# OmerMersin/video-stab

Hardware: AMD Instinct MI355X
Metric: stabilized frames/sec @1080p (whole job; warp-stage HBM GB/s in roofline) (higher is better)
Workload: dtype u8

## Files before the change

### video-stab_amd/csrc/batch_schedule.cpp

```cpp
#include <cstring>
#include <new>

#include "stab_internal.h"

using namespace vsd;

struct vs_batch {
    int device = 0, S = 0, B = 0, cap = 0;
    bool own = false;
    std::vector<vs_stab*> m;
    vs_stab* ref = nullptr;
    std::string err;
    FirstFailure failure;
    hipStream_t st = nullptr, st_pre = nullptr, st_det = nullptr, st_up = nullptr;
    bool allocated = false;
    uint8_t* h_tables = nullptr;
    size_t h_set_bytes = 0, ho_pairs = 0, ho_lk = 0, ho_rs = 0, ho_tail = 0, ho_gf = 0, ho_seg = 0;
    uint8_t* d_all = nullptr;
    uint8_t *d_lk[2] = {nullptr, nullptr}, *d_rs[2] = {nullptr, nullptr}, *d_tail[2] = {nullptr, nullptr}, *d_seg[2] = {nullptr, nullptr}, *d_gf = nullptr;
    uint8_t* d_tin[2] = {nullptr, nullptr};
    ImgPair* d_pairs[2] = {nullptr, nullptr};
    size_t up_bytes = 0;
    int pre_rel_step = -1;
    double* d_MinvB[2] = {nullptr, nullptr};
    int32_t* d_tabs[2] = {nullptr, nullptr};
    int tab_ints = 0;
    hipEvent_t ev_bpre = nullptr, ev_bgray = nullptr, ev_bnms = nullptr, ev_bdet[4] = {}, ev_blk[4] = {}, ev_warp[2] = {}, ev_rel[2] = {}, ev_up[2] = {}, ev_go = nullptr;
    bool bdet_valid[4] = {false, false, false, false}, warp_valid[2] = {false, false}, rel_valid[2] = {false, false};
    int last_det_batch = -1, last_warp_set = -1, batch_id = 0, pend_set = 0;
    struct Ready {
        bool valid = false, tabs_built = false;
        int n = 0, set = 0, step = -1;
        size_t stride = 0;
        std::vector<const uint8_t*> srcs;
        std::vector<uint8_t*> dsts;
        std::vector<int> slots, pad_idx;
        std::vector<vs_stab*> owner;
    };
    static constexpr int NRQ = WARP_LAG + 1;
    Ready rq[NRQ];
    int rq_head = 0, rq_n = 0;
    Ready& pending(int i) { return rq[(rq_head + i) % NRQ]; }
    Ready& building() { return rq[(rq_head + rq_n) % NRQ]; }
    void pop_pending() { rq_head = (rq_head + 1) % NRQ; rq_n--; }

    struct HostSet { uint8_t* base; ImgPair* pairs; uint8_t *lk, *rs, *tail, *seg, *gf; };
    HostSet host_set(int k) const {
        uint8_t* b = h_tables + (size_t)(k % 4) * h_set_bytes;
        return {b, reinterpret_cast<ImgPair*>(b + ho_pairs), b + ho_lk, b + ho_rs, b + ho_tail, b + ho_seg, b + ho_gf};
    }
    int dev_set(int k) const { return k & 1; }
    hipEvent_t blk_event(int k) const { return ev_blk[k % 4]; }
    hipEvent_t det_event(int k) const { return ev_bdet[k % 4]; }
    bool& det_valid(int k) { return bdet_valid[k % 4]; }
    static_assert(WARP_LAG >= 1 && WARP_LAG <= 2, "d_MinvB / d_tabs / ev_warp / ev_rel: two sets cover a lag of at most two steps");
    void flip_pend_set() { pend_set ^= 1; }
    bool warps_due(int k) { return rq_n > 0 && pending(0).step <= k - WARP_LAG; }

    template <typename F>
    void each_event(F f) {
        for (hipEvent_t* e : {&ev_bpre, &ev_bgray, &ev_bnms, &ev_warp[0], &ev_warp[1], &ev_rel[0], &ev_rel[1], &ev_up[0], &ev_up[1], &ev_go}) f(*e);
        for (auto& e : ev_bdet) f(e);
        for (auto& e : ev_blk) f(e);
    }
};

namespace {

void group_free(vs_batch* g) {
    if (g->h_tables) (void)hipHostFree(g->h_tables);
    if (g->d_all) (void)hipFree(g->d_all);
    g->h_tables = nullptr; g->d_all = nullptr;
    g->allocated = false;
    g->ref = nullptr;
}

bool group_make_events(vs_batch* g) {
    bool ok = true;
    g->each_event([&](hipEvent_t& e) { ok = ok && hipEventCreateWithFlags(&e, hipEventDisableTiming) == hipSuccess; });
    return ok;
}

static bool same_yuv_pad(const vs_stab* a, const vs_stab* b) {
    const bool on = yuv_pad_on(a);
    if (on != yuv_pad_on(b)) return false;
    if (!on) return true;
    const vs_yuv_fill x = yuv_pad_fill(a), y = yuv_pad_fill(b);
    return x.y == y.y && x.u == y.u && x.v == y.v;
}
static bool same_yuv_edge_fill(const vs_stab* a, const vs_stab* b) {
    const bool on = yuv_edge_fill_on(a);
    if (on != yuv_edge_fill_on(b)) return false;
    if (!on) return true;
    const vs_yuv_fill x = yuv_edge_fill(a), y = yuv_edge_fill(b);
    return x.y == y.y && x.u == y.u && x.v == y.v;
}
bool same_launch_shape(const vs_stab* a, const vs_stab* b) {
    const vs_params_c &p = a->p, &q = b->p;
    return a->w == b->w && a->h == b->h && a->fmt == b->fmt && a->src_pitch == b->src_pitch && a->zero_copy == b->zero_copy &&
           a->in == b->in && a->out == b->out && a->yuv_cz == b->yuv_cz && same_yuv_pad(a, b) && same_yuv_edge_fill(a, b) &&
           a->aw == b->aw && a->ah == b->ah && a->levels == b->levels &&
           p.lk_win_size == q.lk_win_size && p.ransac_max_iters == q.ransac_max_iters && p.border_size == q.border_size &&
           p.crop_n_zoom == q.crop_n_zoom && (p.border_size <= 0 || p.border_type == q.border_type);
}

int group_allocate(vs_batch* g) {
    const vs_stab* s0 = g->ref;
    const int cap = g->cap, ngf = g->S * (g->B / 2 + 1);
    size_t off = 0;
    auto take = [&](size_t bytes) { size_t o = off; off += (bytes + 255) & ~(size_t)255; return o; };
    const size_t o_gf = take(gftt_item_bytes() * ngf);
    size_t ho = 0;
    auto htake = [&](size_t bytes) { size_t o = ho; ho += (bytes + 255) & ~(size_t)255; return o; };
    g->ho_pairs = htake(sizeof(ImgPair) * cap * MAX_PYR);
    g->ho_lk = htake(lk_item_bytes() * cap); g->ho_rs = htake(ransac_item_bytes() * cap);
    g->ho_tail = htake(tail_item_bytes() * cap); g->ho_seg = htake(tail_seg_bytes() * g->S);
    g->up_bytes = ho;
    g->ho_gf = htake(gftt_item_bytes() * ngf);
    g->h_set_bytes = ho;
    const size_t o_set[2] = {take(g->up_bytes), take(g->up_bytes)};
    const size_t o_ti[2] = {take(tail_in_bytes() * cap), take(tail_in_bytes() * cap)};
    const size_t o_minv[2] = {take((size_t)cap * 96), take((size_t)cap * 96)};
    int tow, toh;
    out_size(s0, s0->w, s0->h, &tow, &toh);
    g->tab_ints = s0->pf->three_planes() ? planar_tab_ints(tow, toh, s0->pf->sx, s0->pf->sy) : s0->pf->luma_uv() ? nv12_tab_ints(tow, toh) : (int)warp_tabs_ints(std::max(s0->w, tow), std::max(s0->h, toh), 1);
    size_t o_tabs[2];
    for (auto& o : o_tabs) o = take((size_t)g->tab_ints * cap * sizeof(int32_t));
    VS_OBJ_HIP(g, hipMalloc((void**)&g->d_all, off));
    VS_OBJ_HIP(g, hipMemsetAsync(g->d_all, 0, off, g->st));
    uint8_t* b = g->d_all;
    g->d_gf = b + o_gf;
    for (int i = 0; i < 2; i++) {
        uint8_t* ds = b + o_set[i];
        g->d_pairs[i] = (ImgPair*)(ds + g->ho_pairs);
        g->d_lk[i] = ds + g->ho_lk; g->d_rs[i] = ds + g->ho_rs; g->d_tail[i] = ds + g->ho_tail; g->d_seg[i] = ds + g->ho_seg; g->d_tin[i] = b + o_ti[i];
        g->d_MinvB[i] = (double*)(b + o_minv[i]);
    }
    for (int i = 0; i < 2; i++) g->d_tabs[i] = (int32_t*)(b + o_tabs[i]);
    VS_OBJ_HIP(g, hipHostMalloc((void**)&g->h_tables, 4 * ho));
    memset(g->h_tables, 0, 4 * ho);
    VS_OBJ_HIP(g, hipStreamSynchronize(g->st));
    for (vs_batch::Ready& r : g->rq) {
        r.srcs.assign(cap, nullptr); r.dsts.assign(cap, nullptr); r.slots.assign(cap, -1); r.pad_idx.assign(cap, 0); r.owner.assign(cap, nullptr);
    }
    g->allocated = true;
    return VS_OK;
}

struct WarpEnds { const uint8_t* src; uint8_t* dst; };
WarpEnds warp_ends(const vs_stab* o, const uint8_t* frame, uint8_t* d_out, int pad_idx, const BorderPlan& bp) {
    if (!bp.pad && !bp.crop) return {frame, d_out};
    return bp.pad ? WarpEnds{scratch(o, pad_idx), d_out} : WarpEnds{frame, scratch(o, pad_idx)};
}

int group_ready_launches(vs_batch* g, vs_batch::Ready& R, int what, hipStream_t st) {
    const vs_stab* s0 = g->ref;
    const BorderPlan bp = border_plan(s0);
    const bool cz = yuv_cz_on(s0);
    const bool yp = yuv_pad_on(s0);
    const YuvBorder wb = s0->pf->kind != PIX_INTERLEAVED ? yuv_warp_border(s0) : YuvBorder{VS_BORDER_BLACK, WarpFill()};
    int rc = VS_OK;
    for (int i0 = 0; i0 < R.n && rc == VS_OK; i0 += WARP_BATCH_MAX) {
        const int m = std::min(WARP_BATCH_MAX, R.n - i0);
        const uint8_t* srcs[WARP_BATCH_MAX];
        uint8_t* dsts[WARP_BATCH_MAX];
        for (int i = 0; i < m; i++) {
            const WarpEnds e = warp_ends(R.owner[i0 + i], R.srcs[i0 + i], R.dsts[i0 + i], R.pad_idx[i0 + i], bp);
            srcs[i] = e.src; dsts[i] = e.dst;
            if (bp.pad && !yp && what != VS_WARP_TABLES_ONLY && rc == VS_OK)
                rc = launch_make_border(R.srcs[i0 + i], s0->src_pitch, s0->w, s0->h, s0->cn, const_cast<uint8_t*>(e.src), bp.prow, bp.b, s0->p.border_type, st);
        }
        if (yp && what != VS_WARP_TABLES_ONLY && rc == VS_OK) rc = pad_launch(s0, &R.srcs[i0], const_cast<uint8_t* const*>(srcs), m, st);
        if (rc != VS_OK) break;
        const WarpMaps maps{g->d_MinvB[R.set] + 12 * i0, 12, false};
        const WarpTabs tabs{WarpTabs::CALLER, g->d_tabs[R.set] + (size_t)i0 * g->tab_ints, g->tab_ints, what};
        if (s0->pf->kind != PIX_INTERLEAVED) {
            rc = warp_yuv(srcs, dsts, m, warp_src_planes(s0), warp_dst_planes(s0, dsts[0], R.stride), maps, wb, tabs, st);
            if (cz && what != VS_WARP_TABLES_ONLY && rc == VS_OK) rc = cz_launch(s0, dsts, &R.dsts[i0], m, R.stride, st);
            continue;
        }
        rc = launch_warp_plane(srcs, dsts, m, bp.pad ? bp.prow : s0->src_pitch, bp.pw, bp.ph, bp.crop ? bp.prow : R.stride, bp.pw, bp.ph, s0->cn, maps,
                               VS_BORDER_BLACK, tabs, st);
        for (int i = 0; bp.crop && what != VS_WARP_TABLES_ONLY && i < m && rc == VS_OK; i++)
            rc = launch_resize_linear(dsts[i] + ((size_t)bp.b * s0->w + bp.b) * s0->cn, bp.prow, s0->w - 2 * bp.b, s0->h - 2 * bp.b, s0->cn,
                                      R.dsts[i0 + i], R.stride, R.owner[i0 + i]->orig_w, R.owner[i0 + i]->orig_h, st);
    }
    if (rc != VS_OK) g->err = get_last_error();
    return rc;
}

int group_launch_ready(vs_batch* g, hipEvent_t det_done = nullptr) {
    if (g->rq_n == 0) return VS_OK;
    vs_batch::Ready& R = g->pending(0);
    hipStream_t st = g->st_pre;
    int rc;
    if (g->rel_valid[R.set] || det_done) {
        hipError_t e = hipSuccess;
        if (WARP_LAG >= 2) {
            if (g->rel_valid[R.set]) e = hipStreamWaitEvent(st, g->ev_rel[R.set], 0);
            if (e == hipSuccess && det_done) e = hipStreamWaitEvent(st, det_done, 0);
        } else {
            if (det_done) e = hipStreamWaitEvent(g->st_up, det_done, 0);
            if (e == hipSuccess && g->rel_valid[R.set]) e = hipStreamWaitEvent(g->st_up, g->ev_rel[R.set], 0);
            if (e == hipSuccess) e = hipEventRecord(g->ev_go, g->st_up);
            if (e == hipSuccess) e = hipStreamWaitEvent(st, g->ev_go, 0);
        }
        if (e != hipSuccess) return vs_obj_fail(g, VS_ERR_HIP, "hipStreamWaitEvent failed");
        if (g->rel_valid[R.set]) g->pre_rel_step = std::max(g->pre_rel_step, R.step);
        g->rel_valid[R.set] = false;
    }
    {
        StageScope t(g->ref, VS_STAGE_WARP, st);
        rc = group_ready_launches(g, R, R.tabs_built ? VS_WARP_ONLY : VS_WARP_ALL, st);
    }
    const hipError_t ew = hipEventRecord(g->ev_warp[R.set], st);
    if (ew == hipSuccess) { g->warp_valid[R.set] = true; g->last_warp_set = R.set; }
    else if (rc == VS_OK) rc = hip_fail(ew, "hipEventRecord(g->ev_warp[R.set], st)");
    for (int i = 0; i < R.n; i++) {
        if (!R.owner[i]) continue;
        const int rrc = release_slot(R.owner[i], R.slots[i], st);
        if (rc == VS_OK) rc = rrc;
    }
    R.valid = false;
    g->pop_pending();
    if (rc != VS_OK) g->err = get_last_error();
    return rc;
}


struct StepPlan {
    int k = 0;
    int n = 0, max_n = 0;
    int n_max = 0;
    int ndet = 0;
    int npend = 0, nseg = 0;
    int aligned = 1;
    int any_apart = 0, all_apart = 1;
    size_t pend_stride = 0;
};

int fill_stream_items(vs_batch* g, vs_stab* s, const vs_batch::HostSet& H, const BorderPlan& bp, int ndue, int first, StepPlan& P) {
    const vs_params_c& p = s->p;
    const int ns = (int)s->bq.size(), dset = g->dev_set(P.k), set = g->pend_set;
    vs_batch::Ready& R = g->building();
    int npad = 0;
    for (int i = 0; i < ns; i++) {
        const int idx = first + i;
        const vs_stab::BFrame& b = s->bq[i];
        const vs_stab::ItemBufs& it = s->items[i];
        LKLevel L[MAX_PYR];
        fill_lk_levels(s, b.pv, b.c, L);
        const int cap = std::max(b.lk_cap, 0);
        P.n_max = std::max(P.n_max, cap);
        uint8_t *rs = H.rs + ransac_item_bytes() * idx, *tail = H.tail + tail_item_bytes() * idx;
        VS_OBJ_TRY(g, lk_fill_item(H.lk + lk_item_bytes() * idx, L, s->levels, s->d_pts[b.lk_buf], cap, s->d_npts[b.lk_buf], it.next, it.status, it.err,
                              p.lk_win_size, p.lk_max_iters, p.lk_epsilon));
        VS_OBJ_TRY(g, ransac_fill_item(rs, s->d_pts[b.lk_buf], it.next, it.status, cap, s->d_npts[b.lk_buf], it.vp, it.vc, it.m, 4, p.ransac_threshold,
                                  p.ransac_max_iters, s->tab, it.counts, it.model, it.inliers, it.info, s->d_traj, &s->tp, s->d_dbg, b.have_prev_gray));
        ransac_item_set_last(rs, i == ns - 1 ? 1 : 0);
        ransac_item_set_tail_in(rs, g->d_tin[dset] + tail_in_bytes() * idx);
        double* minv = nullptr;
        WarpTabJob jobs[2] = {{nullptr, nullptr, nullptr, 0, 0}, {nullptr, nullptr, nullptr, 0, 0}};
        if (b.out_due) {
            const int j = P.npend++;
            minv = g->d_MinvB[set] + 12 * j;
            R.srcs[j] = b.out_frame; R.dsts[j] = b.d_out; R.slots[j] = b.out_slot; R.owner[j] = s; R.pad_idx[j] = npad;
            if (P.all_apart && std::min(WARP_BATCH_MAX, ndue - j / WARP_BATCH_MAX * WARP_BATCH_MAX) >= WARP_TAB_MIN) {
                const WarpEnds e = warp_ends(s, b.out_frame, b.d_out, npad, bp);
                int32_t* T = g->d_tabs[set] + (size_t)j * g->tab_ints;
                jobs[0] = WarpTabJob{T, e.src, e.dst, bp.pw, bp.ph};
                if (s->pf->kind != PIX_INTERLEAVED) {
                    const Planes S = warp_src_planes(s), D = warp_dst_planes(s, e.dst, b.out_stride);
                    jobs[1] = WarpTabJob{T + tab_layout(bp.pw, bp.ph).stride, e.src + S[1].off, e.dst + D[1].off, S[1].w, S[1].h};
                }
            }
            npad++;
            P.pend_stride = b.out_stride;
        }
        tail_fill_item(tail, b.out_due ? 1 : 0, b.out_idx, minv, jobs);
        tail_item_set_seg(tail, P.nseg);
    }
    tail_fill_seg(H.seg + tail_seg_bytes() * P.nseg, first, ns, s->d_M, s->d_traj, s->d_dbg, p.smoothing_method);
    P.any_apart |= p.smoothing_method != VS_SMOOTH_KALMAN;
    P.nseg++;
    return VS_OK;
}

void fill_pair_tables(const vs_batch* g, const std::vector<vs_stab*>& act, ImgPair* h_pairs, StepPlan& P) {
    const int L = g->ref->levels;
    int n_first = 0, n_rest = 0, i = 0;
    for (vs_stab* s : act)
        for (const vs_stab::BFrame& b : s->bq) {
            const Pyramid& py = s->pyr[b.c];
            const int slot = b.detect ? n_first++ : P.ndet + n_rest++;
            h_pairs[slot] = ImgPair{b.frame, py.img[0]};
            if ((uintptr_t)b.frame % 8) P.aligned = 0;
            for (int l = 1; l <= L; l++) h_pairs[(size_t)l * P.n + i] = ImgPair{py.img[l - 1], py.img[l]};
            i++;
        }
}

int fill_detector_items(vs_batch* g, const std::vector<vs_stab*>& act, uint8_t* h_gf) {
    int ndet = 0;
    for (vs_stab* s : act) {
        int local = 0;
        for (const vs_stab::BFrame& b : s->bq) {
            if (!b.detect) continue;
            VS_OBJ_TRY(g, gftt_fill_item(h_gf + gftt_item_bytes() * ndet, s->pyr[b.c].img[0], s->aw, s->aw, s->ah, s->pts_cap[b.det_buf], 0.02, 15.0, 3,
                                    s->gws[local], s->d_pts[b.det_buf], s->d_npts[b.det_buf]));
            s->dbg_det_pts = s->d_pts[b.det_buf]; s->dbg_det_n = s->d_npts[b.det_buf];
            s->dbg_gftt_counters = s->gws[local].counters;
            local++; ndet++;
        }
        s->last_detected = s->bq.back().detect;
    }
    return VS_OK;
}

int step_fill_tables(vs_batch* g, const std::vector<vs_stab*>& act, StepPlan& P) {
    const vs_batch::HostSet H = g->host_set(P.k);
    int ndue = 0;
    for (vs_stab* s : act) {
        for (const vs_stab::BFrame& b : s->bq) { ndue += b.out_due ? 1 : 0; P.ndet += b.detect ? 1 : 0; }
        if (s->p.smoothing_method == VS_SMOOTH_KALMAN) P.all_apart = 0;
    }
    const BorderPlan bp = border_plan(g->ref);
    int first = 0;
    for (vs_stab* s : act) {
        VS_OBJ_TRY(g, fill_stream_items(g, s, H, bp, ndue, first, P));
        first += (int)s->bq.size();
    }
    fill_pair_tables(g, act, H.pairs, P);
    return fill_detector_items(g, act, H.gf);
}

int step_issue_pre(vs_batch* g, const std::vector<vs_stab*>& act, const StepPlan& P, bool warps_go) {
    const vs_stab* s0 = g->ref;
    const int k = P.k, n = P.n, dset = g->dev_set(k);
    hipStream_t pre = g->st_pre;
    if (k >= PYR_STEPS && g->pre_rel_step < k - PYR_STEPS) {
        VS_OBJ_HIP(g, hipStreamWaitEvent(pre, g->blk_event(k - PYR_STEPS), 0));
        if (g->det_valid(k - PYR_STEPS)) VS_OBJ_HIP(g, hipStreamWaitEvent(pre, g->det_event(k - PYR_STEPS), 0));
    }
    for (vs_stab* s : act)
        if (s->bq[0].prev_small) {
            StageScope t(g->ref, VS_STAGE_PYRAMID, pre);
            VS_OBJ_TRY(g, launch_resize_gray(s->d_first_gray, 480, 480, 270, VS_FMT_GRAY8, s->pyr[s->bq[0].pv].img[0], s->aw, s->aw, s->ah, pre));
            VS_OBJ_TRY(g, build_pyramid(s, s->bq[0].pv, pre));
        }
    ImgPair* const d_pairs = g->d_pairs[dset];
    if (k >= 2) VS_OBJ_HIP(g, hipStreamWaitEvent(g->st_up, g->blk_event(k - 2), 0));
    VS_OBJ_HIP(g, hipMemcpyAsync(d_pairs, g->host_set(k).base, g->up_bytes, hipMemcpyHostToDevice, g->st_up));
    VS_OBJ_HIP(g, hipEventRecord(g->ev_up[dset], g->st_up));
    VS_OBJ_HIP(g, hipStreamWaitEvent(pre, g->ev_up[dset], 0));
    {
        StageScope t(g->ref, VS_STAGE_GRAY, pre);
        const int gfmt = s0->pf->gray_source;
        const int n_a = (P.ndet > 0 && P.ndet < n) ? P.ndet : n;
        VS_OBJ_TRY(g, launch_resize_gray_batch(d_pairs, n_a, s0->src_pitch, s0->w, s0->h, gfmt, s0->aw, s0->aw, s0->ah, P.aligned, pre));
        VS_OBJ_HIP(g, hipEventRecord(g->ev_bgray, pre));
        if (n_a < n)
            VS_OBJ_TRY(g, launch_resize_gray_batch(d_pairs + n_a, n - n_a, s0->src_pitch, s0->w, s0->h, gfmt, s0->aw, s0->aw, s0->ah, P.aligned, pre));
    }
    {
        StageScope t(g->ref, VS_STAGE_PYRAMID, pre);
        for (int l = 0; l < s0->levels; l++)
            VS_OBJ_TRY(g, launch_pyr_level_batch(nullptr, d_pairs + (size_t)(l + 1) * n, n, s0->lw[l], s0->lw[l], s0->lh[l], s0->lw[l + 1], pre));
    }
    if (!warps_go) VS_OBJ_HIP(g, hipEventRecord(g->ev_bpre, pre));
    return VS_OK;
}

int step_issue_det(vs_batch* g, const StepPlan& P) {
    const vs_stab* s0 = g->ref;
    const int k = P.k, ndet = P.ndet;
    hipStream_t sd = g->st_det;
    g->det_valid(k) = ndet > 0;
    if (ndet == 0) return VS_OK;
    VS_OBJ_HIP(g, hipMemcpyAsync(g->d_gf, g->host_set(k).gf, gftt_item_bytes() * ndet, hipMemcpyHostToDevice, sd));
    if (k >= 2) VS_OBJ_HIP(g, hipStreamWaitEvent(sd, g->blk_event(k - 2), 0));
    VS_OBJ_TRY(g, launch_gftt_batch(g->d_gf, ndet, s0->aw, s0->ah, 3, sd, 1));
    VS_OBJ_HIP(g, hipStreamWaitEvent(sd, g->ev_bgray, 0));
    {
        StageScope t(g->ref, VS_STAGE_GFTT, sd);
        VS_OBJ_TRY(g, launch_gftt_batch(g->d_gf, ndet, s0->aw, s0->ah, 3, sd, 4));
        VS_OBJ_TRY(g, launch_gftt_batch(g->d_gf, ndet, s0->aw, s0->ah, 3, sd, 5));
        VS_OBJ_HIP(g, hipEventRecord(g->ev_bnms, sd));
        VS_OBJ_TRY(g, launch_gftt_batch(g->d_gf, ndet, s0->aw, s0->ah, 3, sd, 3));
    }
    VS_OBJ_HIP(g, hipEventRecord(g->det_event(k), sd));
    g->last_det_batch = k;
    return VS_OK;
}

int step_issue_main(vs_batch* g, const std::vector<vs_stab*>& act, const StepPlan& P, bool warps_go, int kd) {
    const vs_stab* s0 = g->ref;
    const int dset = g->dev_set(P.k), set = g->pend_set;
    hipStream_t st = g->st;
    if (warps_go && g->last_warp_set >= 0) VS_OBJ_HIP(g, hipStreamWaitEvent(st, g->ev_warp[g->last_warp_set], 0));
    else VS_OBJ_HIP(g, hipStreamWaitEvent(st, g->ev_bpre, 0));
    for (vs_stab* s : act)
        if (s->pts_pending[0]) { VS_OBJ_HIP(g, hipStreamWaitEvent(st, s->pts_event[0], 0)); s->pts_pending[0] = false; }
    if (kd >= 0) VS_OBJ_HIP(g, hipStreamWaitEvent(st, g->det_event(kd), 0));
    {
        StageScope t(g->ref, VS_STAGE_LK, st);
        VS_OBJ_TRY(g, launch_pyr_lk_batch(g->d_lk[dset], P.n, P.n_max, s0->p.lk_win_size, st));
    }
    {
        StageScope t(g->ref, VS_STAGE_RANSAC, st);
        VS_OBJ_TRY(g, launch_ransac_score_batch(g->d_rs[dset], P.n, s0->p.ransac_max_iters, P.n_max, st));
    }
    for (vs_stab* s : act)
        if (s->dbg_delay_us > 0) { VS_OBJ_TRY(g, launch_spin(s->dbg_delay_us, st)); break; }
    if (P.npend > 0 && g->warp_valid[set]) {
        VS_OBJ_HIP(g, hipStreamWaitEvent(st, g->ev_warp[set], 0));
        g->warp_valid[set] = false;
    }
    {
        StageScope t(g->ref, VS_STAGE_TRAJ, st);
        VS_OBJ_TRY(g, launch_ransac_tail_group(g->d_rs[dset], g->d_tail[dset], g->d_seg[dset], g->d_tin[dset], P.nseg, P.max_n, P.n, P.any_apart, st));
    }
    VS_OBJ_HIP(g, hipEventRecord(g->blk_event(P.k), st));
    return VS_OK;
}

int step_publish(vs_batch* g, const std::vector<vs_stab*>& act, const StepPlan& P) {
    const int set = g->pend_set;
    vs_batch::Ready& R = g->building();
    R.n = P.npend; R.set = set; R.stride = P.pend_stride; R.valid = P.npend > 0; R.tabs_built = P.all_apart != 0; R.step = P.k;
    if (R.valid) {
        g->rq_n++;
        g->flip_pend_set();
        if (!R.tabs_built) {
            StageScope t(g->ref, VS_STAGE_WARP_TABLES, g->st);
            VS_OBJ_TRY(g, group_ready_launches(g, R, VS_WARP_TABLES_ONLY, g->st));
            R.tabs_built = true;
        }
        VS_OBJ_HIP(g, hipEventRecord(g->ev_rel[set], g->st));
        g->rel_valid[set] = true;
    }
    for (vs_stab* s : act) {
        const vs_stab::BFrame& lb = s->bq.back();
        const int nl = (int)s->bq.size();
        s->dbg_prev_pts = s->d_pts[lb.lk_buf]; s->dbg_next = s->items[nl - 1].next;
        s->dbg_status = s->items[nl - 1].status; s->dbg_inliers = s->items[nl - 1].inliers;
        s->bq.clear();
    }
    return VS_OK;
}

int group_step(vs_batch* g, const std::vector<vs_stab*>& act, int n, int max_n, int k) {
    StepPlan P;
    P.k = k; P.n = n; P.max_n = max_n;
    if (k >= 4) VS_OBJ_HIP(g, hipEventSynchronize(g->blk_event(k - 4)));
    VS_OBJ_TRY(g, step_fill_tables(g, act, P));
    const bool warps_go = g->warps_due(k);
    VS_OBJ_TRY(g, step_issue_pre(g, act, P, warps_go));
    VS_OBJ_TRY(g, step_issue_det(g, P));
    const int kd = (g->last_det_batch >= 0 && g->last_det_batch >= k - 1) ? g->last_det_batch : -1;
    const hipEvent_t det_done = kd == k ? g->ev_bnms : (kd >= 0 ? g->det_event(kd) : (hipEvent_t) nullptr);
    while (g->warps_due(k)) VS_OBJ_TRY(g, group_launch_ready(g, det_done));
    VS_OBJ_TRY(g, step_issue_main(g, act, P, warps_go, kd));
    return step_publish(g, act, P);
}

}

bool group_holds_warps(const vs_batch* g) { return g && g->rq_n > 0; }

const FirstFailure& group_failure(const vs_batch* g) { return g->failure; }

int group_run(vs_batch* g) {
    if (g->failure.rc != VS_OK) return vs_obj_fail(g, g->failure.rc, g->failure.msg);
    std::vector<vs_stab*> act;
    int n = 0, max_n = 0;
    for (vs_stab* s : g->m)
        if (!s->bq.empty()) { act.push_back(s); n += (int)s->bq.size(); max_n = std::max(max_n, (int)s->bq.size()); }
    if (n == 0) return VS_OK;
    VS_OBJ_HIP(g, hipSetDevice(g->device));
    const vs_stab* s0 = g->ref ? g->ref : act[0];
    size_t out_stride = 0;
    int ndue = 0;
    for (vs_stab* s : act) {
        if (!s->allocated || !s->batch_active || !same_launch_shape(s, s0))
            return vs_obj_fail(g, VS_ERR_INVALID_ARG, "vs_batch: the streams of a group share one frame geometry, pitch, input mode and launch shape "
                                                "(analysis size, pyramid depth, tracking window, hypothesis count, border mode)");
        for (const vs_stab::BFrame& b : s->bq) {
            if (!b.out_due) continue;
            if (ndue++ > 0 && out_stride != b.out_stride) return vs_obj_fail(g, VS_ERR_INVALID_ARG, "batch mode: one output pitch per step");
            out_stride = b.out_stride;
        }
    }
    if (n > g->cap || max_n > BATCH_MAX) return vs_obj_fail(g, VS_ERR_CAPACITY, "vs_batch: more frames queued than a step holds");
    if (!g->allocated) {
        g->ref = act[0];
        const int rc = group_allocate(g);
        if (rc != VS_OK) { group_free(g); return rc; }
    }
    const int rc = group_step(g, act, n, max_n, g->batch_id++);
    g->failure.note(rc, g->err);
    return rc;
}

int group_drain(vs_batch* g) {
    VS_OBJ_HIP(g, hipSetDevice(g->device));
    VS_OBJ_TRY(g, group_run(g));
    int rc = VS_OK;
    while (g->rq_n > 0 && rc == VS_OK) rc = group_launch_ready(g);
    g->failure.note(rc, g->err);
    return rc;
}

void group_delete(vs_batch* g) {
    if (!g) return;
    group_free(g);
    g->each_event([](hipEvent_t& e) { if (e) { (void)hipEventDestroy(e); e = nullptr; } });
    delete g;
}

vs_batch* group_new_own(vs_stab* s) {
    vs_batch* g = new (std::nothrow) vs_batch();
    if (!g) { set_last_error("out of host memory"); return nullptr; }
    g->device = s->device; g->S = 1; g->B = s->batch; g->cap = s->batch; g->own = true;
    g->m.push_back(s);
    g->st = s->st; g->st_pre = s->st_pre; g->st_det = s->st_det; g->st_up = s->st_warp;
    if (!group_make_events(g)) { set_last_error("hipEventCreate failed"); group_delete(g); return nullptr; }
    return g;
}

namespace {
struct MemberCall {
    vs_stab* s;
    explicit MemberCall(vs_stab* s_) : s(s_) { s->group_call = true; }
    ~MemberCall() { s->group_call = false; }
};
}

extern "C" {

static int batch_create(int device, int n_streams, const vs_params_c* params, int per_stream, int frames_per_step, vs_batch** out) {
    if (!out) return VS_ERR_INVALID_ARG;
    *out = nullptr;
    if (!params || n_streams < 1 || n_streams > 256 || frames_per_step < 1 || frames_per_step > BATCH_MAX) {
        set_last_error("vs_batch_create: 1..256 streams, 1..64 frames per stream and step");
        return VS_ERR_INVALID_ARG;
    }
    for (int i = 0; i < (per_stream ? n_streams : 1); i++) {
        const vs_params_c& p = params[i];
        if (p.struct_size != (int32_t)sizeof(vs_params_c)) { set_last_error("params: struct_size mismatch"); return VS_ERR_INVALID_ARG; }
        if (p.adaptive_smoothing || (p.border_size > 0 && !p.crop_n_zoom && p.border_type == VS_BORDER_FADE) || (p.enable_virtual_canvas && !p.crop_n_zoom)) {
            set_last_error("vs_batch_create: adaptive smoothing, the fade border and the virtual canvas are per-stream modes (use vs_stab_*)");
            return VS_ERR_UNSUPPORTED;
        }
    }
    vs_batch* g = new (std::nothrow) vs_batch();
    if (!g) return VS_ERR_HIP;
    g->device = device; g->S = n_streams; g->B = frames_per_step; g->cap = n_streams * frames_per_step;
    for (int i = 0; i < n_streams; i++) {
        vs_stab* s = nullptr;
        int rc = vs_stab_create(&params[per_stream ? i : 0], device, &s);
        if (rc == VS_OK) rc = vs_stab_set_batch(s, frames_per_step);
        if (rc != VS_OK) { if (s) vs_stab_destroy(s); vs_batch_destroy(g); return rc; }
        s->group = g; s->member = true;
        g->m.push_back(s);
    }
    g->st = g->m[0]->st; g->st_pre = g->m[0]->st_pre; g->st_det = g->m[0]->st_det; g->st_up = g->m[0]->st_warp;
    if (!group_make_events(g)) { set_last_error("vs_batch_create: hipEventCreate failed"); vs_batch_destroy(g); return VS_ERR_HIP; }
    *out = g;
    return VS_OK;
}

int vs_batch_create(int device, int n_streams, const vs_params_c* params, int frames_per_step, vs_batch** out) {
    return batch_create(device, n_streams, params, 0, frames_per_step, out);
}

int vs_batch_create_params(int device, int n_streams, const vs_params_c* params_per_stream, int frames_per_step, vs_batch** out) {
    return batch_create(device, n_streams, params_per_stream, 1, frames_per_step, out);
}

void vs_batch_destroy(vs_batch* g) {
    if (!g) return;
    (void)hipSetDevice(g->device);
    (void)sync_streams({g->st_pre, g->st_det, g->st});
    for (vs_stab* s : g->m) { s->group = nullptr; s->member = false; s->bq.clear(); vs_stab_destroy(s); }
    group_delete(g);
}

int vs_batch_streams(const vs_batch* g) { return g ? g->S : 0; }
vs_stab* vs_batch_stream(vs_batch* g, int i) { return (g && i >= 0 && i < g->S) ? g->m[(size_t)i] : nullptr; }
const char* vs_batch_last_error(const vs_batch* g) { return g ? g->err.c_str() : ""; }

int vs_batch_set_zero_copy(vs_batch* g, int enable) {
    if (!g) return VS_ERR_INVALID_ARG;
    for (vs_stab* s : g->m) { MemberCall mc(s); const int rc = vs_stab_set_zero_copy(s, enable); if (rc != VS_OK) { g->err = s->err; return rc; } }
    return VS_OK;
}

int vs_batch_set_nv12_layout(vs_batch* g, size_t in_uv_offset, size_t out_uv_offset) {
    if (!g) return VS_ERR_INVALID_ARG;
    for (vs_stab* s : g->m) { MemberCall mc(s); const int rc = vs_stab_set_nv12_layout(s, in_uv_offset, out_uv_offset); if (rc != VS_OK) { g->err = s->err; return rc; } }
    return VS_OK;
}

int vs_batch_set_i420_layout(vs_batch* g, size_t in_u_off, size_t in_v_off, size_t in_c_pitch, size_t out_u_off, size_t out_v_off, size_t out_c_pitch) {
    if (!g) return VS_ERR_INVALID_ARG;
    for (vs_stab* s : g->m) {
        MemberCall mc(s);
        const int rc = vs_stab_set_i420_layout(s, in_u_off, in_v_off, in_c_pitch, out_u_off, out_v_off, out_c_pitch);
        if (rc != VS_OK) { g->err = s->err; return rc; }
    }
    return VS_OK;
}

int vs_batch_set_yuv_crop_zoom(vs_batch* g, int enable) {
    if (!g) return VS_ERR_INVALID_ARG;
    for (vs_stab* s : g->m) { MemberCall mc(s); const int rc = vs_stab_set_yuv_crop_zoom(s, enable); if (rc != VS_OK) { g->err = s->err; return rc; } }
    return VS_OK;
}

int vs_batch_set_yuv_border_pad(vs_batch* g, int enable, const vs_yuv_fill* fill) {
    if (!g) return VS_ERR_INVALID_ARG;
    for (vs_stab* s : g->m) { MemberCall mc(s); const int rc = vs_stab_set_yuv_border_pad(s, enable, fill); if (rc != VS_OK) { g->err = s->err; return rc; } }
    return VS_OK;
}

int vs_batch_set_yuv_edge_fill(vs_batch* g, int enable, const vs_yuv_fill* fill) {
    if (!g) return VS_ERR_INVALID_ARG;
    for (vs_stab* s : g->m) { MemberCall mc(s); const int rc = vs_stab_set_yuv_edge_fill(s, enable, fill); if (rc != VS_OK) { g->err = s->err; return rc; } }
    return VS_OK;
}

int vs_batch_push_dev(vs_batch* g, const void* const* d_frames, int w, int h, size_t stride, int fmt, void* const* d_outs, size_t out_stride,
                      int* produced) {
    if (!g || !d_frames || !d_outs || !produced) return VS_ERR_INVALID_ARG;
    for (int i = 0; i < g->S; i++) produced[i] = 0;
    if (g->failure.rc != VS_OK) return vs_obj_fail(g, g->failure.rc, g->failure.msg);
    bool full = false;
    for (int i = 0; i < g->S; i++) {
        if (!d_frames[i]) continue;
        vs_stab* s = g->m[(size_t)i];
        MemberCall mc(s);
        const int rc = vs_stab_push_dev(s, d_frames[i], w, h, stride, fmt, d_outs[i], out_stride, &produced[i]);
        if (rc != VS_OK) { g->err = s->err; return rc; }
        full |= (int)s->bq.size() >= g->B;
    }
    if (full) return group_run(g);
    return VS_OK;
}

int vs_batch_flush_dev(vs_batch* g, void* const* d_outs, size_t out_stride, int* produced) {
    if (!g || !d_outs || !produced) return VS_ERR_INVALID_ARG;
    int rc = group_drain(g);
    if (rc != VS_OK) return rc;
    for (int i = 0; i < g->S; i++) {
        produced[i] = 0;
        MemberCall mc(g->m[(size_t)i]);
        rc = vs_stab_flush_dev(g->m[(size_t)i], d_outs[i], out_stride, &produced[i]);
        if (rc != VS_OK) { g->err = g->m[(size_t)i]->err; return rc; }
    }
    return VS_OK;
}

int vs_batch_sync(vs_batch* g) {
    if (!g) return VS_ERR_INVALID_ARG;
    int rc = group_drain(g);
    if (rc != VS_OK) return rc;
    for (vs_stab* s : g->m) { rc = vs_stab_sync(s); if (rc != VS_OK) { g->err = s->err; return rc; } }
    return VS_OK;
}

}
```

Baseline: 144,900.

## Triple-buffer per-step device upload sets to loosen upload-to-LK dependency

Raises the number of device-side per-step table sets (pairs, LK, RANSAC, tail, tail input) from two to three and indexes them by k modulo three. The upload stream now only waits for the LK stage from three steps back instead of two before overwriting a set, so the host-to-device copy can run further ahead of the consumers. It costs one more set of device memory, and destroy now also synchronizes the upload stream. Scratch A/B scripts are added alongside.

```diff
diff --git a/scratch/r31_ab_summary.py b/scratch/r31_ab_summary.py
--- /dev/null
+++ b/scratch/r31_ab_summary.py
@@ -0,0 +1,17 @@
+import glob, json, statistics, sys
+d, libs = sys.argv[1], sys.argv[2:]
+def line(p):
+    b = json.loads(open(p).read().strip().splitlines()[-1])
+    return (b["ms_per_step"], b["value"], b["roofline"]["frac"], b["configs"]["configs[2]"]["nv12_stabilize"]["value"], b["outputs_checked"])
+rows = {n: [line(p) for p in sorted(glob.glob("%s/%s_*.json" % (d, n)))] for n in libs}
+def mr(v, f): return (f + " (" + f + " - " + f + ")") % (statistics.median(v), min(v), max(v))
+print("| library | runs | `ms_per_step` | `value` (frames/s) | warp `roofline.frac` | `configs[2].nv12_stabilize.value` | `outputs_checked` |")
+print("|---|---|---|---|---|---|---|")
+for n in libs:
+    r = rows[n]
+    print("| `%s` | %d | %s | %s | %s | %s | %s |" % (n, len(r), mr([x[0] for x in r], "%.4f"), mr([x[1] for x in r], "%.0f"), mr([x[2] for x in r], "%.4f"),
+                                                  mr([x[3] for x in r], "%.0f"), sorted(set(x[4] for x in r))))
+print()
+for n in libs:
+    for i, x in enumerate(rows[n]):
+        print("%-8s run %d: ms_per_step %.4f value %.1f warp_frac %.4f configs2_nv12 %.1f outputs_checked %d" % ((n, i + 1) + x))
diff --git a/scratch/r31_gray_variants.py b/scratch/r31_gray_variants.py
--- /dev/null
+++ b/scratch/r31_gray_variants.py
@@ -0,0 +1,41 @@
+import glob
+import os
+import subprocess
+
+ROOT = os.path.dirname(os.path.dirname(os.path.abspath(__file__)))
+CS = os.path.join(ROOT, "video-stab_amd", "csrc")
+LABS = os.path.join(ROOT, "scratch", "labs")
+GATE = "    if (g->gate_step == k - 1) VS_OBJ_HIP(g, hipStreamWaitEvent(up, g->ev_gate[g->gate_set], 0));\n"
+DETW = "    if (g->last_warp_set >= 0) VS_OBJ_HIP(g, hipStreamWaitEvent(sd, g->ev_warp[g->last_warp_set], 0));\n"
+ONE = """        VS_OBJ_TRY(g, launch_resize_gray_batch(d_pairs, n, s0->src_pitch, s0->w, s0->h, gfmt, s0->aw, s0->aw, s0->ah, P.aligned, up));  // :448-450
+    }
+    VS_OBJ_HIP(g, hipEventRecord(g->ev_bgray, up));     // the analysis images exist: the detector and the pyramid levels wait for it
+    VS_OBJ_HIP(g, hipStreamWaitEvent(pre, g->ev_bgray, 0));
+"""
+TWO = """        const int n_a = (P.ndet > 0 && P.ndet < n) ? P.ndet : n;
+        VS_OBJ_TRY(g, launch_resize_gray_batch(d_pairs, n_a, s0->src_pitch, s0->w, s0->h, gfmt, s0->aw, s0->aw, s0->ah, P.aligned, up));
+        VS_OBJ_HIP(g, hipEventRecord(g->ev_bgray, up));
+        if (n_a < n)
+            VS_OBJ_TRY(g, launch_resize_gray_batch(d_pairs + n_a, n - n_a, s0->src_pitch, s0->w, s0->h, gfmt, s0->aw, s0->aw, s0->ah, P.aligned, up));
+    }
+    VS_OBJ_HIP(g, hipEventRecord(g->ev_go, up));
+    VS_OBJ_HIP(g, hipStreamWaitEvent(pre, g->ev_go, 0));
+"""
+EDITS = {"pr": ("", ""), "free": (GATE, ""), "detfree": (DETW, ""), "split": (ONE, TWO)}
+FLAGS = "-x hip -O3 -std=c++17 -fPIC --offload-arch=gfx950 -ffp-contract=off -fno-fast-math -w".split()
+
+os.makedirs(os.path.join(LABS, "r31_pr"), exist_ok=True)
+PR = os.path.join(LABS, "r31_pr", "batch_schedule.cpp")
+subprocess.check_call(["patch", "-s", "-o", PR, os.path.join(CS, "batch_schedule.cpp"), os.path.join(ROOT, "scratch", "r31_gray_early.patch.txt")])
+src = open(PR).read()
+objs = [o for o in glob.glob(os.path.join(CS, "_build", "*.o")) if not o.endswith("batch_schedule.cpp.o")]
+for name, (old, new) in EDITS.items():
+    assert not old or src.count(old) == 1, name
+    d = os.path.join(LABS, "r31_" + name)
+    os.makedirs(d, exist_ok=True)
+    if old:
+        open(os.path.join(d, "batch_schedule.cpp"), "w").write(src.replace(old, new))
+    obj = os.path.join(d, "batch_schedule.o")
+    subprocess.check_call(["/opt/rocm/bin/hipcc"] + FLAGS + ["-I" + CS, "-I" + os.path.join(ROOT, "include"), "-c", os.path.join(d, "batch_schedule.cpp"), "-o", obj])
+    subprocess.check_call(["/opt/rocm/bin/hipcc", "-shared", "-fPIC", "--offload-arch=gfx950", "-o", os.path.join(LABS, "libvs_%s.so" % name), obj] + objs)
+    print("built", name)
diff --git a/scratch/r31_headline.py b/scratch/r31_headline.py
--- /dev/null
+++ b/scratch/r31_headline.py
@@ -0,0 +1,8 @@
+import glob, subprocess, sys, os
+out, header, jobs = sys.argv[1], sys.argv[2], [a.split(":") for a in sys.argv[3:]]
+here = os.path.dirname(os.path.abspath(__file__))
+with open(out, "w") as f:
+    f.write(open(header).read())
+    for d, libs in jobs:
+        f.write("\n## job %s, order of a round: %s\n" % (os.path.basename(d), " ".join(libs.split(","))))
+        f.write(subprocess.check_output([sys.executable, os.path.join(here, "r31_ab_summary.py"), d] + libs.split(",")).decode())
diff --git a/video-stab_amd/csrc/batch_schedule.cpp b/video-stab_amd/csrc/batch_schedule.cpp
--- a/video-stab_amd/csrc/batch_schedule.cpp
+++ b/video-stab_amd/csrc/batch_schedule.cpp
@@ -17,15 +17,16 @@
     uint8_t* h_tables = nullptr;
     size_t h_set_bytes = 0, ho_pairs = 0, ho_lk = 0, ho_rs = 0, ho_tail = 0, ho_gf = 0, ho_seg = 0;
     uint8_t* d_all = nullptr;
-    uint8_t *d_lk[2] = {nullptr, nullptr}, *d_rs[2] = {nullptr, nullptr}, *d_tail[2] = {nullptr, nullptr}, *d_seg[2] = {nullptr, nullptr}, *d_gf = nullptr;
-    uint8_t* d_tin[2] = {nullptr, nullptr};
-    ImgPair* d_pairs[2] = {nullptr, nullptr};
+    static constexpr int DEV_SETS = 3;
+    uint8_t *d_lk[DEV_SETS] = {}, *d_rs[DEV_SETS] = {}, *d_tail[DEV_SETS] = {}, *d_seg[DEV_SETS] = {}, *d_gf = nullptr;
+    uint8_t* d_tin[DEV_SETS] = {};
+    ImgPair* d_pairs[DEV_SETS] = {};
     size_t up_bytes = 0;
     int pre_rel_step = -1;
     double* d_MinvB[2] = {nullptr, nullptr};
     int32_t* d_tabs[2] = {nullptr, nullptr};
     int tab_ints = 0;
-    hipEvent_t ev_bpre = nullptr, ev_bgray = nullptr, ev_bnms = nullptr, ev_bdet[4] = {}, ev_blk[4] = {}, ev_warp[2] = {}, ev_rel[2] = {}, ev_up[2] = {}, ev_go = nullptr;
+    hipEvent_t ev_bpre = nullptr, ev_bgray = nullptr, ev_bnms = nullptr, ev_bdet[4] = {}, ev_blk[4] = {}, ev_warp[2] = {}, ev_rel[2] = {}, ev_up[DEV_SETS] = {}, ev_go = nullptr;
     bool bdet_valid[4] = {false, false, false, false}, warp_valid[2] = {false, false}, rel_valid[2] = {false, false};
     int last_det_batch = -1, last_warp_set = -1, batch_id = 0, pend_set = 0;
     struct Ready {
@@ -49,7 +50,7 @@
         uint8_t* b = h_tables + (size_t)(k % 4) * h_set_bytes;
         return {b, reinterpret_cast<ImgPair*>(b + ho_pairs), b + ho_lk, b + ho_rs, b + ho_tail, b + ho_seg, b + ho_gf};
     }
-    int dev_set(int k) const { return k & 1; }
+    int dev_set(int k) const { return k % DEV_SETS; }
     hipEvent_t blk_event(int k) const { return ev_blk[k % 4]; }
     hipEvent_t det_event(int k) const { return ev_bdet[k % 4]; }
     bool& det_valid(int k) { return bdet_valid[k % 4]; }
@@ -59,7 +60,8 @@
 
     template <typename F>
     void each_event(F f) {
-        for (hipEvent_t* e : {&ev_bpre, &ev_bgray, &ev_bnms, &ev_warp[0], &ev_warp[1], &ev_rel[0], &ev_rel[1], &ev_up[0], &ev_up[1], &ev_go}) f(*e);
+        for (hipEvent_t* e : {&ev_bpre, &ev_bgray, &ev_bnms, &ev_warp[0], &ev_warp[1], &ev_rel[0], &ev_rel[1], &ev_go}) f(*e);
+        for (auto& e : ev_up) f(e);
         for (auto& e : ev_bdet) f(e);
         for (auto& e : ev_blk) f(e);
     }
@@ -118,8 +120,9 @@
     g->up_bytes = ho;
     g->ho_gf = htake(gftt_item_bytes() * ngf);
     g->h_set_bytes = ho;
-    const size_t o_set[2] = {take(g->up_bytes), take(g->up_bytes)};
-    const size_t o_ti[2] = {take(tail_in_bytes() * cap), take(tail_in_bytes() * cap)};
+    size_t o_set[vs_batch::DEV_SETS], o_ti[vs_batch::DEV_SETS];
+    for (auto& o : o_set) o = take(g->up_bytes);
+    for (auto& o : o_ti) o = take(tail_in_bytes() * cap);
     const size_t o_minv[2] = {take((size_t)cap * 96), take((size_t)cap * 96)};
     int tow, toh;
     out_size(s0, s0->w, s0->h, &tow, &toh);
@@ -130,13 +133,12 @@
     VS_OBJ_HIP(g, hipMemsetAsync(g->d_all, 0, off, g->st));
     uint8_t* b = g->d_all;
     g->d_gf = b + o_gf;
-    for (int i = 0; i < 2; i++) {
+    for (int i = 0; i < vs_batch::DEV_SETS; i++) {
         uint8_t* ds = b + o_set[i];
         g->d_pairs[i] = (ImgPair*)(ds + g->ho_pairs);
         g->d_lk[i] = ds + g->ho_lk; g->d_rs[i] = ds + g->ho_rs; g->d_tail[i] = ds + g->ho_tail; g->d_seg[i] = ds + g->ho_seg; g->d_tin[i] = b + o_ti[i];
-        g->d_MinvB[i] = (double*)(b + o_minv[i]);
-    }
-    for (int i = 0; i < 2; i++) g->d_tabs[i] = (int32_t*)(b + o_tabs[i]);
+    }
+    for (int i = 0; i < 2; i++) { g->d_MinvB[i] = (double*)(b + o_minv[i]); g->d_tabs[i] = (int32_t*)(b + o_tabs[i]); }
     VS_OBJ_HIP(g, hipHostMalloc((void**)&g->h_tables, 4 * ho));
     memset(g->h_tables, 0, 4 * ho);
     VS_OBJ_HIP(g, hipStreamSynchronize(g->st));
@@ -349,7 +351,7 @@
             VS_OBJ_TRY(g, build_pyramid(s, s->bq[0].pv, pre));
         }
     ImgPair* const d_pairs = g->d_pairs[dset];
-    if (k >= 2) VS_OBJ_HIP(g, hipStreamWaitEvent(g->st_up, g->blk_event(k - 2), 0));
+    if (k >= vs_batch::DEV_SETS) VS_OBJ_HIP(g, hipStreamWaitEvent(g->st_up, g->blk_event(k - vs_batch::DEV_SETS), 0));
     VS_OBJ_HIP(g, hipMemcpyAsync(d_pairs, g->host_set(k).base, g->up_bytes, hipMemcpyHostToDevice, g->st_up));
     VS_OBJ_HIP(g, hipEventRecord(g->ev_up[dset], g->st_up));
     VS_OBJ_HIP(g, hipStreamWaitEvent(pre, g->ev_up[dset], 0));
@@ -581,7 +583,7 @@
 void vs_batch_destroy(vs_batch* g) {
     if (!g) return;
     (void)hipSetDevice(g->device);
-    (void)sync_streams({g->st_pre, g->st_det, g->st});
+    (void)sync_streams({g->st_up, g->st_pre, g->st_det, g->st});
     for (vs_stab* s : g->m) { s->group = nullptr; s->member = false; s->bq.clear(); vs_stab_destroy(s); }
     group_delete(g);
 }
```

New measurement: 144,300, median of 2. No clear change (-0.4%).
